# tud-amr/m3p2i-aip

Measured on AMD Instinct MI355X. Metric: mppi_state_steps_per_sec (K x T per command()), higher is better.
Workload: dtype f32; 1 GPU; point_env task=push goal=[-1.0, -1.0] K=2000 (2000/GPU) T=30 single-mode halton-spline, initial scene, open loop (fixed world, warm-started plan); parallelism=single GPU

## Files before the change

### include/m3p2i_hip.h

```cpp
#ifndef M3P2I_HIP_H
#define M3P2I_HIP_H

#ifdef __cplusplus
extern "C" {
#endif

#define M3_MAX_NU 9
#define M3_TOPK 20
#define M3_ABI_VERSION 4

typedef enum {
    M3_OK = 0,
    M3_ERR_BAD_ARG = -1,
    M3_ERR_HIP = -2,
    M3_ERR_SHAPE = -3,
    M3_ERR_STATE = -4,
    M3_ERR_UNSUPPORTED = -5
} m3_status;

typedef enum { M3_ENV_POINT = 0, M3_ENV_PANDA = 1 } m3_env;

typedef enum {
    M3_TASK_NAVIGATION = 0,
    M3_TASK_PUSH = 1,
// ... 86 lines not shown
    M3_BUF_PENDING_FORCE = 19,
    M3_BUF_INFO = 20,
    M3_BUF_SIM_WORLD = 21,
    M3_BUF_RECORD = 22,
    M3_BUF_RECORDS_ALL = 23,
    M3_BUF_NOISE_ALL = 24,
    M3_BUF_COV = 25,
    M3_BUF_RECORD_B = 26,
    M3_BUF_RECORDS_B_ALL = 27,
    M3_BUF_COUNT = 28
} m3_buffer_id;

typedef struct m3_handle m3_handle;

int m3_abi_version(void);
const char* m3_last_error(const m3_handle* h);
const char* m3_build_id(void);
void m3_default_config(m3_config* cfg, int env_type);
int m3_create(const m3_config* cfg, m3_handle** out);
void m3_destroy(m3_handle* h);
int m3_set_stream(m3_handle* h, void* hip_stream);
int m3_enable_timing(m3_handle* h, int on);
int m3_set_rollout_lanes(m3_handle* h, int lanes);
int m3_set_panda_lanes_per_sample(m3_handle* h, int lanes_per_sample);
int m3_set_panda_reach_cost_kernel(m3_handle* h, int on);
int m3_panda_lanes_per_sample_used(m3_handle* h);
int m3_panda_near_share(m3_handle* h);
int m3_set_update_launches(m3_handle* h, int launches);

int m3_set_wave_order(m3_handle* h, int on);
int m3_set_ladder_spins(m3_handle* h, int spins);
int m3_relabel_samples(m3_handle* h);

int m3_set_noise(m3_handle* h, const float* delta, int on_device);
int m3_set_noise_knots(m3_handle* h, const float* knots, int n_knots, int degree, float smoothing,
                       int on_device);
int m3_set_noise_global(m3_handle* h, const float* delta_all, int on_device);
int m3_set_noise_knots_global(m3_handle* h, const float* knots_all, int n_knots, int degree, float smoothing,
                              int on_device);
int m3_set_noise_halton(m3_handle* h, int n_knots, int degree, float smoothing);
#define M3_HALTON_PLAIN 0
#define M3_HALTON_FAURE 1
int m3_set_noise_halton_scrambled(m3_handle* h, int n_knots, int degree, float smoothing, int scramble);
int m3_sample_noise(m3_handle* h);
int m3_set_objective(m3_handle* h, int task, const float* goal, int goal_len, int gripper_cmd);
int m3_set_avoid_dyn_obs(m3_handle* h, int on);
// ... 137 lines not shown
```

### m3p2i_aip_amd/_lib.py

```python
from __future__ import annotations

import ctypes as C
import os

MAX_NU = 9
TOPK = 20
ABI_VERSION = 4

_HERE = os.path.dirname(os.path.abspath(__file__))
LIB_PATH = os.environ.get("M3P2I_HIP_LIB") or os.path.join(_HERE, "lib", "libm3p2i_hip.so")

ENV_POINT, ENV_PANDA = 0, 1
HALTON_PLAIN, HALTON_FAURE = 0, 1
IPC_HANDLE_BYTES = 64
TASKS = {"navigation": 0, "push": 1, "pull": 2, "push_pull": 3, "reach": 4, "pick": 5,
         "place": 6, "idle": 7}

(BUF_STATES, BUF_ACTIONS, BUF_COST_HORIZON, BUF_TRAJ_COST, BUF_TRAJ_COST_ALL, BUF_WEIGHTS,
 BUF_WEIGHTS_1, BUF_WEIGHTS_2, BUF_MEAN, BUF_MEAN_1, BUF_MEAN_2, BUF_BEST, BUF_BEST_1,
 BUF_BEST_2, BUF_ACTION_OUT, BUF_TOP_IDX, BUF_TOP_TRAJS, BUF_REDUCE, BUF_NOISE,
 BUF_PENDING_FORCE, BUF_INFO, BUF_SIM_WORLD, BUF_RECORD, BUF_RECORDS_ALL, BUF_NOISE_ALL, BUF_COV,
 BUF_RECORD_B, BUF_RECORDS_B_ALL, BUF_COUNT) = range(29)


# ... 57 lines not shown

PE_RUNNING, PE_SETTLING, PE_FROZEN = 0, 1, 2
PANDA_EPISODE_TRACE_FLOATS = 132
PE_TR_DOF, PE_TR_ROOT, PE_TR_ACTION, PE_TR_HAND, PE_TR_CUBE = 0, 18, 109, 118, 125


class Timing(C.Structure):
    _fields_ = [("rollout_ms", C.c_float), ("update_ms", C.c_float),
                ("finalize_ms", C.c_float), ("total_ms", C.c_float)]


_H = C.c_void_p
_FP = C.c_void_p
SYMBOLS = [
    ("m3_abi_version", C.c_int, []),
    ("m3_build_id", C.c_char_p, []),
    ("m3_last_error", C.c_char_p, [_H]),
    ("m3_default_config", None, [C.POINTER(Config), C.c_int]),
    ("m3_create", C.c_int, [C.POINTER(Config), C.POINTER(_H)]),
    ("m3_destroy", None, [_H]),
    ("m3_set_stream", C.c_int, [_H, C.c_void_p]),
    ("m3_enable_timing", C.c_int, [_H, C.c_int]),
    ("m3_set_rollout_lanes", C.c_int, [_H, C.c_int]),
    ("m3_set_panda_lanes_per_sample", C.c_int, [_H, C.c_int]),
    ("m3_panda_lanes_per_sample_used", C.c_int, [_H]),
    ("m3_panda_near_share", C.c_int, [_H]),
    ("m3_set_panda_reach_cost_kernel", C.c_int, [_H, C.c_int]),
    ("m3_set_update_launches", C.c_int, [_H, C.c_int]),
    ("m3_set_ladder_spins", C.c_int, [_H, C.c_int]),
    ("m3_set_wave_order", C.c_int, [_H, C.c_int]),
    ("m3_relabel_samples", C.c_int, [_H]),
    ("m3_set_noise", C.c_int, [_H, _FP, C.c_int]),
    ("m3_set_noise_knots", C.c_int, [_H, _FP, C.c_int, C.c_int, C.c_float, C.c_int]),
    ("m3_set_noise_global", C.c_int, [_H, _FP, C.c_int]),
    ("m3_set_noise_knots_global", C.c_int, [_H, _FP, C.c_int, C.c_int, C.c_float, C.c_int]),
    ("m3_set_noise_halton", C.c_int, [_H, C.c_int, C.c_int, C.c_float]),
    ("m3_set_noise_halton_scrambled", C.c_int, [_H, C.c_int, C.c_int, C.c_float, C.c_int]),
    ("m3_sample_noise", C.c_int, [_H]),
    ("m3_set_call_count", C.c_int, [_H, C.c_uint]),
    ("m3_set_objective", C.c_int, [_H, C.c_int, C.POINTER(C.c_float), C.c_int, C.c_int]),
    ("m3_set_avoid_dyn_obs", C.c_int, [_H, C.c_int]),
    ("m3_default_point_cost_weights", None, [C.POINTER(PointCostWeights)]),
    ("m3_set_point_cost_weights", C.c_int, [_H, C.POINTER(PointCostWeights)]),
    ("m3_get_point_cost_weights", C.c_int, [_H, C.POINTER(PointCostWeights)]),
    ("m3_set_weighted_cost_instance", C.c_int, [_H, C.c_int]),
    ("m3_set_multi_modal", C.c_int, [_H, C.c_int]),
# ... 104 lines not shown
```

### m3p2i_aip_amd/csrc/m3_api.hip

```cpp
#include <algorithm>
#include <cmath>
#include <cstddef>
#include <cstdio>
#include <cstdlib>
#include <cstring>
#include <tuple>
#include <vector>
#include <new>

#include "m3_internal.hpp"
#include "panda_episode_lane.hpp"

using namespace m3;

static thread_local std::string g_create_err;

#define HIPCHK(o, expr)                                                                  \
    do {                                                                                 \
        hipError_t e_ = (expr);                                                          \
        if (e_ != hipSuccess) {                                                          \
            (o)->err = std::string(#expr) + ": " + hipGetErrorString(e_);                \
            return M3_ERR_HIP;                                                           \
        }                                                                                \
    } while (0)
// ... 238 lines not shown
        if (hipMalloc((void**)&h->wave_min, (size_t)Kl * 3 * f) != hipSuccess) rc = M3_ERR_HIP;
        if (rc == M3_OK && hipMalloc((void**)&h->lflag, nl * sizeof(int)) != hipSuccess) rc = M3_ERR_HIP;
        if (rc == M3_OK && hipMemset(h->lflag, 0, nl * sizeof(int)) != hipSuccess) rc = M3_ERR_HIP;
    }
    if (rc == M3_OK && c->env_type == M3_ENV_PANDA) {
        void* p = nullptr;
        void* q = nullptr;
        void* d = nullptr;
        if (hipHostMalloc(&p, sizeof(int), hipHostMallocMapped) != hipSuccess || hipMalloc(&q, sizeof(unsigned long long)) != hipSuccess ||
            hipMemset(q, 0, sizeof(unsigned long long)) != hipSuccess || hipHostGetDevicePointer(&d, p, 0) != hipSuccess) {
            if (p) (void)hipHostFree(p);
            if (q) (void)hipFree(q);
            h->err = "m3_create: the panda rollout's report word (mapped host memory) could not be allocated";
            rc = M3_ERR_HIP;
        } else {
            h->panda_busy_hint = (int*)p;
            h->panda_busy_hint_dev = (int*)d;
            h->panda_busy_count = (unsigned long long*)q;
            *h->panda_busy_hint = 0;
        }
        if (rc == M3_OK && Kl == Kg && Kg >= 2 && Kl <= PANDA_REACH_REC_MAX_K &&
            hipMalloc((void**)&h->panda_reach_rec, (size_t)T * REACH_REC * (size_t)Kl * f) != hipSuccess) rc = M3_ERR_HIP;
    }
    if (rc == M3_OK && hipMalloc((void**)&h->wcount, (size_t)(T + 2) * sizeof(int)) != hipSuccess) rc = M3_ERR_HIP;
    if (rc == M3_OK && hipMemset(h->wcount, 0, (size_t)(T + 2) * sizeof(int)) != hipSuccess) rc = M3_ERR_HIP;
    if (rc == M3_OK) {
        m3_info init;
        std::memset(&init, 0, sizeof(init));
        init.beta = init.beta_1 = init.beta_2 = 1.0f;
        if (hipMemcpy(h->buf[M3_BUF_INFO], &init, sizeof(init), hipMemcpyHostToDevice) != hipSuccess) rc = M3_ERR_HIP;
    }
    if (rc != M3_OK) {
        g_create_err = h->err.empty() ? "m3_create: device allocation failed" : h->err;
        m3_destroy(h);
        return rc;
    }
    (void)hipDeviceSynchronize();
    *out = h;
    return M3_OK;
}

extern "C" void m3_destroy(m3_handle* h) {
    if (!h) return;
    if (h->regen) h->buf[M3_BUF_TRAJ_COST] = h->buf[M3_BUF_NOISE] = h->buf[M3_BUF_NOISE_ALL] = nullptr;
    for (int i = 0; i < M3_BUF_COUNT; ++i)
        if (h->buf[i]) (void)hipFree(h->buf[i]);
    if (h->noise_all) (void)hipFree(h->noise_all);
    if (h->noise_mats) (void)hipFree(h->noise_mats);
    if (h->local_top_idx) (void)hipFree(h->local_top_idx);
    if (h->world0_dev) (void)hipFree(h->world0_dev);
    if (h->topk_cand) (void)hipFree(h->topk_cand);
    if (h->part_min) (void)hipFree(h->part_min);
    if (h->lad) (void)hipFree(h->lad);
    if (h->wpart) (void)hipFree(h->wpart);
    if (h->apart) (void)hipFree(h->apart);
    if (h->wcount) (void)hipFree(h->wcount);
    if (h->wave_min) (void)hipFree(h->wave_min);
    if (h->lflag) (void)hipFree(h->lflag);
    if (h->sim_world) (void)hipFree(h->sim_world);
    if (h->sim_u) (void)hipFree(h->sim_u);
    if (h->noise_stage) (void)hipFree(h->noise_stage);
    if (h->order) (void)hipFree(h->order);
    if (h->order_scratch) (void)hipFree(h->order_scratch);
    if (h->noise_sorted) (void)hipFree(h->noise_sorted);
    for (int p = 0; p < MIX_MAX_RANKS; ++p)
        if (h->peer_ipc[p] && h->peer_base[p]) (void)hipIpcCloseMemHandle(h->peer_base[p]);
    if (h->xb) (void)hipFree(h->xb);
    if (h->panda_busy_hint) (void)hipHostFree(h->panda_busy_hint);
    if (h->panda_busy_count) (void)hipFree(h->panda_busy_count);
    if (h->panda_reach_rec) (void)hipFree(h->panda_reach_rec);
    for (auto& ev : h->ev)
        if (ev) (void)hipEventDestroy(ev);
    delete h;
}

#ifndef M3_BUILD_ID
#define M3_BUILD_ID "unknown"
#endif
extern "C" const char* m3_build_id(void) { return M3_BUILD_ID; }

extern "C" int m3_set_stream(m3_handle* h, void* s) {
    if (!h) return M3_ERR_BAD_ARG;
    h->stream = (hipStream_t)s;
    return M3_OK;
}

extern "C" int m3_set_rollout_lanes(m3_handle* h, int lanes) {
    if (!h) return M3_ERR_BAD_ARG;
    if (lanes != 0 && (lanes < 1 || lanes > 64 || (lanes & (lanes - 1)) != 0))
        return fail(h, M3_ERR_BAD_ARG, "m3_set_rollout_lanes: lanes must be 0 (auto) or a power of two in 1..64");
    h->lanes_override = lanes;
    return M3_OK;
}

extern "C" int m3_set_panda_lanes_per_sample(m3_handle* h, int lps) {
    if (!h) return M3_ERR_BAD_ARG;
    if (lps != 0 && lps != 1 && lps != 8 && lps != 16)
        return fail(h, M3_ERR_BAD_ARG, "m3_set_panda_lanes_per_sample: 0 (by size), 1, 8 or 16");
    h->panda_lps = lps;
    return M3_OK;
}

extern "C" int m3_set_panda_reach_cost_kernel(m3_handle* h, int on) {
    if (!h) return M3_ERR_BAD_ARG;
    h->panda_reach_deferred = on != 0;
    return M3_OK;
}

extern "C" int m3_panda_near_share(m3_handle* h) {
    return (h && h->panda_busy_hint) ? *(volatile const int*)h->panda_busy_hint - 1 : -1;
}

extern "C" int m3_panda_lanes_per_sample_used(m3_handle* h) {
    return h ? h->panda_lps_used : 0;
}
// ... 548 lines not shown
    a.cost_h = (float*)h->buf[M3_BUF_COST_HORIZON];
    a.J = (float*)h->buf[M3_BUF_TRAJ_COST];
    a.wave_min = h->wave_min;
    return M3_OK;
}

static void fill_panda_args(m3_handle* h, const RolloutArgs& a, PandaArgs& pa) {
    std::memcpy(pa.world0, h->pworld0, sizeof(pa.world0));
    pa.cubeA_actor = h->bind_box; pa.cubeB_actor = h->bind_dyn; pa.obs_actor = h->bind_obs;
    fill_panda_cost_params(h, pa.cp);
    pa.shadows = (pa.cp.task == 4 && a.k0 == 0 && a.Kl == a.Kg && a.Kg >= 2) ? (pa.cp.multi_modal ? 2 : 1) : 0;
    pa.lps = h->panda_lps;
    pa.reach_rec = (pa.shadows != 0 && a.Kl <= PANDA_REACH_REC_MAX_K && h->panda_reach_deferred) ? h->panda_reach_rec : nullptr;
    pa.busy_hint = h->panda_busy_hint_dev; pa.busy_count = h->panda_busy_count; pa.reach_busy = 0;
    if (h->panda_busy_hint) {
        const int share = *(volatile const int*)h->panda_busy_hint - 1;
        const int on = pa.reach_rec ? PANDA_BUSY_ON_REC : PANDA_BUSY_ON, off = pa.reach_rec ? PANDA_BUSY_OFF_REC : PANDA_BUSY_OFF;
        if (share >= on) h->panda_reach_busy = 1;
        else if (share >= 0 && share < off) h->panda_reach_busy = 0;
        pa.reach_busy = h->panda_reach_busy;
    }
}

static int plan_rollout(m3_handle* h, RolloutArgs& a, PandaArgs& pa, RolloutPlan& p) {
    const int rc = prepare_rollout(h, a);
    if (rc != M3_OK) return rc;
    if (h->cfg.env_type == M3_ENV_POINT) {
        p = plan_rollout_point(a, h->scene, weighted_cost(h));
    } else {
        fill_panda_args(h, a, pa);
        p = plan_rollout_panda(a, pa);
        h->panda_lps_used = p.lps;
    }
    a.lanes = p.lanes;
    h->wave_min_rows = p.rows;
    return M3_OK;
}

extern "C" int m3_rollout(m3_handle* h) {
    if (!h) return M3_ERR_BAD_ARG;
    if (const char* why = rollout_refusal(h)) return fail(h, M3_ERR_STATE, why);
    RolloutArgs a;
    PandaArgs pa;
    RolloutPlan p;
    const int rc = plan_rollout(h, a, pa, p);
    if (rc != M3_OK) return rc;
    if (h->timing) HIPCHK(h, hipEventRecord(h->ev[0], h->stream));
    if (h->cfg.env_type == M3_ENV_POINT) launch_rollout_point(a, h->scene, h->cost_weights, p, h->stream);
    else launch_rollout_panda(a, pa, h->pscene, p, h->stream);
    HIPCHK(h, hipGetLastError());
    if (h->timing) HIPCHK(h, hipEventRecord(h->ev[1], h->stream));
    return M3_OK;
}

static float* plan_dst(const m3_handle* h) { return h->action_out ? h->action_out : (float*)h->buf[M3_BUF_ACTION_OUT]; }
static size_t plan_floats(const m3_config& c) { return (size_t)(c.mode_simple ? c.u_per_command : c.T) * c.nu; }

static void fill_update_args(m3_handle* h, UpdateArgs& a) {
    const m3_config& c = h->cfg;
    std::memset(&a, 0, sizeof(a));
    a.Kg = c.K_global; a.Kl = c.K_local; a.k0 = c.k_offset; a.T = c.T; a.nu = c.nu;
    a.multi_modal = c.multi_modal; a.mode_simple = c.mode_simple; a.env_type = c.env_type;
    a.filter_u = c.filter_u; a.u_per_command = c.u_per_command;
    a.lambda_ = c.lambda_; a.step_size_mean = c.step_size_mean;
    a.cand = h->topk_cand;
    a.ladder_spins = h->ladder_spins;
    a.p2p_err = (h->p2p_ready && h->xb) ? (const int*)((const char*)h->xb + 2 * MIX_MAX_RANKS * sizeof(int)) : nullptr;
    a.part_min = h->part_min;
    a.n_cand = topk_workgroups(c.K_global);
    a.n_mins = mins_workgroups(c.K_global);
    a.lad = h->lad;
// ... 1441 lines not shown
```

### m3p2i_aip_amd/csrc/m3_internal.hpp

```cpp
#pragma once
#include <hip/hip_runtime.h>

#include <string>

#include "../../include/m3p2i_hip.h"
#include "planar_dyn.hpp"
#include "point_cost.hpp"
#include "panda_dyn.hpp"

namespace m3 {

struct RolloutArgs {
    int Kg, Kl, k0, T, nu;
    int multi_modal, mode_simple, sampling_random, sample_null_action;
    int gripper_cmd;
    float u_min[M3_MAX_NU], u_max[M3_MAX_NU], scale_tril[M3_MAX_NU], sigma_inv[M3_MAX_NU];
    float u_scale, gamma, lambda_;
    int noise_abs_cost, full_sigma;
    float noise_mu[M3_MAX_NU];
    const float* noise_mats;
    const float* scale_dev;
    unsigned long long seed;
    unsigned call;
    CostParams cp;
// ... 104 lines not shown

struct BatchRolloutEntry {
    RolloutArgs a;
    PointScene sc;
};
struct BatchRolloutEntryW {
    RolloutArgs a;
    PointScene sc;
    PointCostWeights wt;
};
struct SmallUpdateInstance {
    int nu, multi, jr, wt, n_cand;
};
SmallUpdateInstance update_small_instance(const UpdateArgs& a);
int update_small_batch_blocks_per_cu(const SmallUpdateInstance& in);
int update_small9_batch_blocks_per_cu(const SmallUpdateInstance& in);
void launch_update_small_batch(const UpdateArgs* tab, int n, const SmallUpdateInstance& in, int T, hipStream_t s);
struct RolloutPlan {
    int instance, ref;
    int lps, forces, general, shadows, rec;
    int lanes, blocks;
    int rows;
    int weighted;
};
RolloutPlan plan_rollout_point(const RolloutArgs& a, const PointScene& sc, bool weighted);
void launch_rollout_point_batch(const BatchRolloutEntry* tab, int n, const RolloutPlan& p, hipStream_t s);
void launch_rollout_point_batch_w(const BatchRolloutEntryW* tab, int n, const RolloutPlan& p, hipStream_t s);
void launch_rollout_point_nav_batch(const BatchRolloutEntry* tab, int blocks, int n, bool ref, hipStream_t s);
void launch_rollout_point_push_batch(const BatchRolloutEntry* tab, int blocks, int n, bool ref, hipStream_t s);
void launch_rollout_point_pull_batch(const BatchRolloutEntry* tab, int blocks, int n, bool ref, hipStream_t s);
void launch_rollout_point_pushpull_batch(const BatchRolloutEntry* tab, int blocks, int n, bool ref, hipStream_t s);

void launch_rollout_point(const RolloutArgs& a, const PointScene& sc, const PointCostWeights& wt ,
                          const RolloutPlan& p, hipStream_t s);
void launch_rollout_point_nav(const RolloutArgs& a, const PointScene& sc, int blocks, hipStream_t s);
void launch_rollout_point_push(const RolloutArgs& a, const PointScene& sc, int blocks, hipStream_t s);
void launch_rollout_point_pull(const RolloutArgs& a, const PointScene& sc, int blocks, hipStream_t s);
void launch_rollout_point_pushpull(const RolloutArgs& a, const PointScene& sc, int blocks, hipStream_t s);
void launch_transpose_noise(const float* src_ktn, float* dst_tkn, int K, int T, int nu,
                            hipStream_t s);
void launch_spline_noise(const float* knots, float* noise, int Kl, int nu, int n_knots, int T, int degree,
                         double smoothing, hipStream_t s);
void launch_sample_noise(const RolloutArgs& a, float* out, hipStream_t s);
void launch_halton_knots(float* knots, int k0, int n, int ncol, const int* primes_dev, const int* perm_dev,
                         const int* perm_off_dev, hipStream_t s);
struct OrderScene {
    const float* sim_root;
    int sim_box, sim_dyn;
    float bx, by, dx, dy;
    float ox, oy;
};
size_t wave_order_temp_bytes(int Kl);
hipError_t launch_wave_order(const float* noise, int Kl, int T, int nu, float s0, float s1, int half_local,
                             const OrderScene& os, void* scratch, size_t temp_bytes, int* order, float* noise_sorted,
                             const int* specials , hipStream_t s);
void launch_gather_rows(const float* src, const int* order, float* dst, int Kl, int rows, hipStream_t s);
void launch_weights(const UpdateArgs& a, hipStream_t s);
void launch_wsum(const UpdateArgs& a, hipStream_t s);
void launch_update_small(const UpdateArgs& a, hipStream_t s);
bool update_small_applies(const UpdateArgs& a);
void launch_finalize(const UpdateArgs& a, hipStream_t s);
void launch_mix(const UpdateArgs& a, hipStream_t s);
void launch_cov_update(const float* actions, const float* w, const float* mean, float* part, float* cov, int K, int T,
                       int nu, hipStream_t s);
void launch_local_topk(const UpdateArgs& a, hipStream_t s);
void launch_regen_fast(const UpdateArgs& a, hipStream_t s);
void launch_p3_search(const UpdateArgs& a, hipStream_t s);
void launch_p3_local_weights(const UpdateArgs& a, hipStream_t s);
void launch_p3_done(const UpdateArgs& a, hipStream_t s);
int init_ladder_table();
int regen_chunks(int Kg);
int rollout_lanes_for(int Kl);
constexpr int M3_CUS = 256;
constexpr int M3_SIMDS = 1024;
inline bool rollout_two_waves(int wavefronts) { return wavefronts > M3_SIMDS; }
inline bool rollout_three_waves(int wavefronts) { return wavefronts > 4 * M3_SIMDS; }
int mins_workgroups(int Kg);
int topk_workgroups(int Kg);
int ladder_workgroups(int Kg);
int wsum_chunks(int Kl);
int apply_workgroups(int Kg);
void launch_mins(const UpdateArgs& a, hipStream_t s);
void launch_ladder(const UpdateArgs& a, hipStream_t s);
void launch_ladder_search(const UpdateArgs& a, hipStream_t s);
void launch_fused_large(const UpdateArgs& a, hipStream_t s);

struct P2PArgs {
    const float* rec;
    int rec_len, rec_stride, n_ranks, rank, slot, seq;
    int plain_memory;
    unsigned long long timeout_ticks;
    int* err;
    float* peer_data[MIX_MAX_RANKS];
    int* peer_flags[MIX_MAX_RANKS];
};
constexpr size_t P2P_HDR_BYTES = 1024;
void launch_p2p_put(const P2PArgs& a, hipStream_t s);
void launch_p2p_wait(const P2PArgs& a, hipStream_t s);
void launch_p2p_exchange(const P2PArgs& a, hipStream_t s);
// ... 108 lines not shown
    int task = M3_TASK_PUSH;
    float goal[7] = {0, 0, 0, 0, 0, 0, 1};
    int gripper_cmd = 0;
    int avoid_dyn_obs = 0;
    m3::PointCostWeights cost_weights = m3::POINT_COST_WEIGHTS_DEFAULT;
    int weighted_instance = -1;
    float world0[18];
    const float* world0_bound = nullptr;
    const float* bind_dof = nullptr;
    const float* bind_root = nullptr;
    int bind_nact = 0, bind_box = 0, bind_dyn = 0, bind_obs = 0;
    bool have_noise = false;
    bool cov_active = false;
    float* noise_mats = nullptr;
    bool regen = false;
    bool regen_fast = false;
    bool p3 = false;
    const float* recb_src = nullptr;
    int recb_stride = 0;
    float* noise_all = nullptr;
    int* local_top_idx = nullptr;
    unsigned calls = 0;
    int lanes_override = 0;
    int* panda_busy_hint = nullptr;
    int* panda_busy_hint_dev = nullptr;
    unsigned long long* panda_busy_count = nullptr;
    float* panda_reach_rec = nullptr;
    bool panda_reach_deferred = true;
    int panda_reach_busy = 0;
    int panda_lps_used = 0;
    int panda_lps = 0;
    void* buf[M3_BUF_COUNT] = {};
    long long nbytes[M3_BUF_COUNT] = {};
    float* world0_dev = nullptr;
    float* action_out = nullptr;
    m3::VI* topk_cand = nullptr;
    float* part_min = nullptr;
    float* lad = nullptr;
    float* wpart = nullptr;
    float* apart = nullptr;
    int* wcount = nullptr;
    float* wave_min = nullptr;
    int wave_min_rows = 0;
    bool use_wave_min = false;
    int* lflag = nullptr;
    int lad_epoch = 0;
// ... 22 lines not shown
```

### m3p2i_aip_amd/csrc/rollout_point.hip

```cpp
#include "rollout_point_kernel.hpp"
#include "episode_lane.hpp"

namespace m3 {

int rollout_lanes_for(int Kl) {
    (void)Kl;
    return 64;
}

__global__ __launch_bounds__(64) void k_rollout_point_w(const RolloutArgs a, const PointScene sc, const PointCostWeights wt) {
    rollout_point_body<true, -1, true, true>(a, sc, &wt);
}
__global__ __launch_bounds__(64) void k_rollout_point_w_ref(const RolloutArgs a, const PointCostWeights wt) {
    constexpr PointScene sc = POINT_SCENE_REFERENCE;
    rollout_point_body<true, -1, true, true>(a, sc, &wt);
}
__global__ __launch_bounds__(64) __attribute__((amdgpu_waves_per_eu(2, 2))) void k_rollout_point_w_occ2(
    const RolloutArgs a, const PointScene sc, const PointCostWeights wt) {
    rollout_point_body<true, -1, false, true>(a, sc, &wt);
}
__global__ __launch_bounds__(64) __attribute__((amdgpu_waves_per_eu(3, 3))) void k_rollout_point_w_occ3(
    const RolloutArgs a, const PointScene sc, const PointCostWeights wt) {
    rollout_point_body<true, -1, false, true>(a, sc, &wt);
}
// ... 11 lines not shown
}
__global__ __launch_bounds__(64) void kb_rollout_point_w_ref(const BatchRolloutEntryW* __restrict__ tab) {
    constexpr PointScene sc = POINT_SCENE_REFERENCE;
    rollout_point_body<true, -1, true, true>(tab[blockIdx.y].a, sc, &tab[blockIdx.y].wt);
}
__global__ __launch_bounds__(64) __attribute__((amdgpu_waves_per_eu(2, 2))) void kb_rollout_point_w_occ2(
    const BatchRolloutEntryW* __restrict__ tab) {
    rollout_point_body<true, -1, false, true>(tab[blockIdx.y].a, tab[blockIdx.y].sc, &tab[blockIdx.y].wt);
}
__global__ __launch_bounds__(64) __attribute__((amdgpu_waves_per_eu(3, 3))) void kb_rollout_point_w_occ3(
    const BatchRolloutEntryW* __restrict__ tab) {
    rollout_point_body<true, -1, false, true>(tab[blockIdx.y].a, tab[blockIdx.y].sc, &tab[blockIdx.y].wt);
}
static void launch_rollout_point_weighted_batch(const BatchRolloutEntryW* tab, int blocks, int n, bool ref, hipStream_t s) {
    const dim3 grid(blocks, n);
    switch (rollout_point_build(blocks * n, ref)) {
        case BUILD_OCC3: hipLaunchKernelGGL(kb_rollout_point_w_occ3, grid, dim3(64), 0, s, tab); break;
        case BUILD_OCC2: hipLaunchKernelGGL(kb_rollout_point_w_occ2, grid, dim3(64), 0, s, tab); break;
        case BUILD_LONE_REF: hipLaunchKernelGGL(kb_rollout_point_w_ref, grid, dim3(64), 0, s, tab); break;
        default: hipLaunchKernelGGL(kb_rollout_point_w, grid, dim3(64), 0, s, tab); break;
    }
}

RolloutPlan plan_rollout_point(const RolloutArgs& a, const PointScene& sc, bool weighted) {
#if defined(M3_ABL_GENERAL_ONLY) || defined(M3_ABL_COUNT) || defined(M3_ABL_PHASES)
    const bool general = true;
#else
    const bool general = a.sampling_random || a.mode_simple || a.cp.task < 0 || a.cp.task > 3 ||
                         (a.cp.task == 3 && !a.multi_modal) || a.scale_dev != nullptr  ||
                         a.cp.avoid_dyn_obs != 0  ||
                         weighted ;
#endif
    RolloutPlan p{};
    p.weighted = weighted ? 1 : 0;
    p.instance = general ? -1 : a.cp.task;
    p.ref = point_scene_is_reference(sc) ? 1 : 0;
    p.lanes = a.lanes;
    p.blocks = (a.Kl + a.lanes - 1) / a.lanes;
    p.rows = (a.wave_min && (p.instance == -1 || p.instance == 3)) ? p.blocks : 0;
    return p;
}

void launch_rollout_point(const RolloutArgs& a, const PointScene& sc, const PointCostWeights& wt, const RolloutPlan& p,
                          hipStream_t s) {
    if (p.weighted) { launch_rollout_point_weighted(a, sc, wt, p.blocks, s); return; }
    switch (p.instance) {
        case -1: launch_rollout_point_instance<true, -1>(a, sc, p.blocks, s); break;
        case 0: launch_rollout_point_nav(a, sc, p.blocks, s); break;
        case 1: launch_rollout_point_push(a, sc, p.blocks, s); break;
        case 2: launch_rollout_point_pull(a, sc, p.blocks, s); break;
        default: launch_rollout_point_pushpull(a, sc, p.blocks, s); break;
    }
}

void launch_rollout_point_batch(const BatchRolloutEntry* tab, int n, const RolloutPlan& p, hipStream_t s) {
    const bool ref = p.ref != 0;
    switch (p.instance) {
        case -1: launch_rollout_point_batch_instance<true, -1>(tab, p.blocks, n, ref, s); break;
        case 0: launch_rollout_point_nav_batch(tab, p.blocks, n, ref, s); break;
        case 1: launch_rollout_point_push_batch(tab, p.blocks, n, ref, s); break;
        case 2: launch_rollout_point_pull_batch(tab, p.blocks, n, ref, s); break;
        default: launch_rollout_point_pushpull_batch(tab, p.blocks, n, ref, s); break;
    }
}

void launch_rollout_point_batch_w(const BatchRolloutEntryW* tab, int n, const RolloutPlan& p, hipStream_t s) {
    launch_rollout_point_weighted_batch(tab, p.blocks, n, p.ref != 0, s);
}
// ... 316 lines not shown
```

### m3p2i_aip_amd/csrc/rollout_point_kernel.hpp

```cpp
#pragma once
#include "m3_internal.hpp"
#include "noise_stream.hpp"
#include "wave_min.hpp"

namespace m3 {

__device__ __forceinline__ void load_world(const float* p, PointWorld& w) {
    w.rx = p[0]; w.ry = p[1]; w.rvx = p[2]; w.rvy = p[3];
    w.B.x = p[4]; w.B.y = p[5]; w.B.c = p[6]; w.B.s = p[7]; w.B.vx = p[8]; w.B.vy = p[9]; w.B.w = p[10];
    w.D.x = p[11]; w.D.y = p[12]; w.D.c = p[13]; w.D.s = p[14]; w.D.vx = p[15]; w.D.vy = p[16]; w.D.w = p[17];
    w.fcDx = w.fcDy = w.fcBx = w.fcBy = w.fcRx = w.fcRy = 0.0f;
}

__device__ __forceinline__ void load_world_from_sim(const float* dof, const float* root, int box,
                                                    int dyn, PointWorld& w) {
    w.rx = dof[0]; w.ry = dof[2]; w.rvx = dof[1]; w.rvy = dof[3];
    const float* r = root + (size_t)box * 13;
    float qz = r[5], qw = r[6];
    w.B.x = r[0]; w.B.y = r[1]; w.B.c = 1.0f - 2.0f * (qz * qz); w.B.s = 2.0f * (qz * qw);
    w.B.vx = r[7]; w.B.vy = r[8]; w.B.w = r[12];
    r = root + (size_t)dyn * 13;
    qz = r[5]; qw = r[6];
    w.D.x = r[0]; w.D.y = r[1]; w.D.c = 1.0f - 2.0f * (qz * qz); w.D.s = 2.0f * (qz * qw);
    w.D.vx = r[7]; w.D.vy = r[8]; w.D.w = r[12];
// ... 142 lines not shown
    rollout_point_body<GENERAL, TASK, false>(a, sc);
}
template <bool GENERAL, int TASK>
__global__ __launch_bounds__(64) __attribute__((amdgpu_waves_per_eu(3, 3))) void k_rollout_point_occ3(const RolloutArgs a,
                                                                                                      const PointScene sc) {
    rollout_point_body<GENERAL, TASK, false>(a, sc);
}
enum RolloutBuild { BUILD_LONE, BUILD_LONE_REF, BUILD_OCC2, BUILD_OCC3 };
inline RolloutBuild rollout_point_build(int waves, bool ref) {
    if (rollout_three_waves(waves)) return BUILD_OCC3;
    if (rollout_two_waves(waves)) return BUILD_OCC2;
    return ref ? BUILD_LONE_REF : BUILD_LONE;
}
template <bool GENERAL, int TASK>
inline void launch_rollout_point_instance(const RolloutArgs& a, const PointScene& sc, int blocks, hipStream_t s) {
    switch (rollout_point_build(blocks, point_scene_is_reference(sc))) {
        case BUILD_OCC3: hipLaunchKernelGGL((k_rollout_point_occ3<GENERAL, TASK>), dim3(blocks), dim3(64), 0, s, a, sc); break;
        case BUILD_OCC2: hipLaunchKernelGGL((k_rollout_point_occ2<GENERAL, TASK>), dim3(blocks), dim3(64), 0, s, a, sc); break;
        case BUILD_LONE_REF: hipLaunchKernelGGL((k_rollout_point_ref<GENERAL, TASK>), dim3(blocks), dim3(64), 0, s, a); break;
        default: hipLaunchKernelGGL((k_rollout_point<GENERAL, TASK>), dim3(blocks), dim3(64), 0, s, a, sc); break;
    }
}

template <bool GENERAL, int TASK>
__global__ __launch_bounds__(64) void kb_rollout_point(const BatchRolloutEntry* __restrict__ tab) {
    rollout_point_body<GENERAL, TASK>(tab[blockIdx.y].a, tab[blockIdx.y].sc);
}
template <bool GENERAL, int TASK>
__global__ __launch_bounds__(64) void kb_rollout_point_ref(const BatchRolloutEntry* __restrict__ tab) {
    constexpr PointScene sc = POINT_SCENE_REFERENCE;
    rollout_point_body<GENERAL, TASK>(tab[blockIdx.y].a, sc);
}
template <bool GENERAL, int TASK>
__global__ __launch_bounds__(64) __attribute__((amdgpu_waves_per_eu(2, 2))) void kb_rollout_point_occ2(
    const BatchRolloutEntry* __restrict__ tab) {
    rollout_point_body<GENERAL, TASK, false>(tab[blockIdx.y].a, tab[blockIdx.y].sc);
}
template <bool GENERAL, int TASK>
__global__ __launch_bounds__(64) __attribute__((amdgpu_waves_per_eu(3, 3))) void kb_rollout_point_occ3(
    const BatchRolloutEntry* __restrict__ tab) {
    rollout_point_body<GENERAL, TASK, false>(tab[blockIdx.y].a, tab[blockIdx.y].sc);
}
template <bool GENERAL, int TASK>
inline void launch_rollout_point_batch_instance(const BatchRolloutEntry* tab, int blocks, int n, bool ref, hipStream_t s) {
    const dim3 grid(blocks, n);
    switch (rollout_point_build(blocks * n, ref)) {
// ... 9 lines not shown
```

### m3p2i_aip_amd/csrc/rollout_point_task0.hip

```cpp
#include "rollout_point_kernel.hpp"

namespace m3 {

void launch_rollout_point_nav(const RolloutArgs& a, const PointScene& sc, int blocks, hipStream_t s) {
    launch_rollout_point_instance<false, 0>(a, sc, blocks, s);
}
void launch_rollout_point_nav_batch(const BatchRolloutEntry* tab, int blocks, int n, bool ref, hipStream_t s) {
    launch_rollout_point_batch_instance<false, 0>(tab, blocks, n, ref, s);
}

}
```

### m3p2i_aip_amd/csrc/rollout_point_task1.hip

```cpp
#include "rollout_point_kernel.hpp"

namespace m3 {

void launch_rollout_point_push(const RolloutArgs& a, const PointScene& sc, int blocks, hipStream_t s) {
    launch_rollout_point_instance<false, 1>(a, sc, blocks, s);
}
void launch_rollout_point_push_batch(const BatchRolloutEntry* tab, int blocks, int n, bool ref, hipStream_t s) {
    launch_rollout_point_batch_instance<false, 1>(tab, blocks, n, ref, s);
}

}
```

### m3p2i_aip_amd/engine.py

```python
from __future__ import annotations

import os

import ctypes as C

import numpy as np
import torch

from . import _lib as L


class _DevArray:

    def __init__(self, ptr, shape, typestr, owner):
        self.__cuda_array_interface__ = {"shape": tuple(shape), "typestr": typestr,
                                         "data": (int(ptr), False), "version": 2}
        self._owner = owner


def make_config(K, T, nu=2, env_type="point_env", multi_modal=False, mode_simple=False,
                sampling_random=False, sample_null_action=True, filter_u=True,
                u_per_command=None, u_min=None, u_max=None, noise_sigma_diag=None, u_scale=1.0,
                gamma=0.95, lambda_=1.0, kp_suction=400.0, pre_height_diff=0.05, dt=None,
                substeps=2, solver_iters=6, seed=0, device=0, K_local=None, k_offset=0,
# ... 41 lines not shown
    c.seed = int(seed)
    return c


class HipEngine:
    def __init__(self, cfg: L.Config):
        if not torch.cuda.is_available():
            raise L.M3Error("HipEngine needs a HIP device (torch.cuda.is_available() is False); "
                            "there is no CPU fallback")
        self.lib = L.load()
        self.cfg = cfg
        self._h = C.c_void_p()
        torch.cuda.set_device(cfg.device)
        torch.zeros(1, device=f"cuda:{cfg.device}")
        L.check(self.lib.m3_create(C.byref(cfg), C.byref(self._h)))
        self.device = torch.device(f"cuda:{cfg.device}")
        self._views = {}
        self._action_out = None
        self.use_torch_stream()
        if os.environ.get("M3P2I_WAVE_ORDER", "1") == "0":
            self.set_wave_order(False)
        if os.environ.get("M3P2I_ROLLOUT_LANES"):
            self.set_rollout_lanes(int(os.environ["M3P2I_ROLLOUT_LANES"]))

    def close(self):
        if getattr(self, "_h", None) is not None and self._h:
            self._views.clear()
            self.lib.m3_destroy(self._h)
            self._h = C.c_void_p()

    def __del__(self):
        try:
            self.close()
        except Exception:
            pass

    def _ck(self, rc):
        L.check(rc, self._h)

    def use_torch_stream(self, stream=None):
        s = stream if stream is not None else torch.cuda.current_stream(self.device)
        self._ck(self.lib.m3_set_stream(self._h, C.c_void_p(s.cuda_stream)))

    def set_rollout_lanes(self, lanes=0):
        self._ck(self.lib.m3_set_rollout_lanes(self._h, int(lanes)))

    def set_panda_lanes_per_sample(self, lps=0):
        self._ck(self.lib.m3_set_panda_lanes_per_sample(self._h, int(lps)))

    def panda_lanes_per_sample_used(self):
        return int(self.lib.m3_panda_lanes_per_sample_used(self._h))

    def set_panda_reach_cost_kernel(self, on=True):
        self._ck(self.lib.m3_set_panda_reach_cost_kernel(self._h, int(bool(on))))

    def panda_near_share(self):
        return int(self.lib.m3_panda_near_share(self._h))

    def set_update_launches(self, launches=0):
        self._ck(self.lib.m3_set_update_launches(self._h, int(launches)))

    def set_ladder_spins(self, spins=-1):
        self._ck(self.lib.m3_set_ladder_spins(self._h, int(spins)))

    def set_wave_order(self, on=True):
        self._ck(self.lib.m3_set_wave_order(self._h, int(bool(on))))

    def relabel_samples(self):
# ... 502 lines not shown
```

Baseline: 512.7 million state-steps/s.

## Split point rollout into producer/consumer wavefronts handing off through LDS

Adds a two-wavefront form of the point-env rollout kernel for navigation and push. One wavefront computes controls and writes actions while the other steps the dynamics serially, and that same control wavefront then evaluates costs and writes states from LDS behind the dynamics wavefront, using atomic progress counters. The aim is to take control construction, cost evaluation and global stores off the serial dynamics chain so they overlap with it. The form is picked automatically when blocks are few (K=2000 here). A mapped-host error word records spin timeouts, which adds a host read per call and a risk of invalid results if a wait runs out.

```diff
diff --git a/include/m3p2i_hip.h b/include/m3p2i_hip.h
--- a/include/m3p2i_hip.h
+++ b/include/m3p2i_hip.h
@@ -132,6 +132,8 @@
 int m3_set_stream(m3_handle* h, void* hip_stream);
 int m3_enable_timing(m3_handle* h, int on);
 int m3_set_rollout_lanes(m3_handle* h, int lanes);
+int m3_set_point_rollout_form(m3_handle* h, int form);
+int m3_point_rollout_form_used(m3_handle* h);
 int m3_set_panda_lanes_per_sample(m3_handle* h, int lanes_per_sample);
 int m3_set_panda_reach_cost_kernel(m3_handle* h, int on);
 int m3_panda_lanes_per_sample_used(m3_handle* h);
diff --git a/m3p2i_aip_amd/_lib.py b/m3p2i_aip_amd/_lib.py
--- a/m3p2i_aip_amd/_lib.py
+++ b/m3p2i_aip_amd/_lib.py
@@ -103,6 +103,8 @@
     ("m3_set_stream", C.c_int, [_H, C.c_void_p]),
     ("m3_enable_timing", C.c_int, [_H, C.c_int]),
     ("m3_set_rollout_lanes", C.c_int, [_H, C.c_int]),
+    ("m3_set_point_rollout_form", C.c_int, [_H, C.c_int]),
+    ("m3_point_rollout_form_used", C.c_int, [_H]),
     ("m3_set_panda_lanes_per_sample", C.c_int, [_H, C.c_int]),
     ("m3_panda_lanes_per_sample_used", C.c_int, [_H]),
     ("m3_panda_near_share", C.c_int, [_H]),
diff --git a/m3p2i_aip_amd/csrc/m3_api.hip b/m3p2i_aip_amd/csrc/m3_api.hip
--- a/m3p2i_aip_amd/csrc/m3_api.hip
+++ b/m3p2i_aip_amd/csrc/m3_api.hip
@@ -284,6 +284,19 @@
         if (rc == M3_OK && Kl == Kg && Kg >= 2 && Kl <= PANDA_REACH_REC_MAX_K &&
             hipMalloc((void**)&h->panda_reach_rec, (size_t)T * REACH_REC * (size_t)Kl * f) != hipSuccess) rc = M3_ERR_HIP;
     }
+    if (rc == M3_OK && c->env_type == M3_ENV_POINT && !c->sim_only) {
+        void* p = nullptr;
+        void* d = nullptr;
+        if (hipHostMalloc(&p, sizeof(int), hipHostMallocMapped) != hipSuccess || hipHostGetDevicePointer(&d, p, 0) != hipSuccess) {
+            if (p) (void)hipHostFree(p);
+            h->err = "m3_create: the point rollout's error word (mapped host memory) could not be allocated";
+            rc = M3_ERR_HIP;
+        } else {
+            h->rollout_err = (int*)p;
+            h->rollout_err_dev = (int*)d;
+            *h->rollout_err = 0;
+        }
+    }
     if (rc == M3_OK && hipMalloc((void**)&h->wcount, (size_t)(T + 2) * sizeof(int)) != hipSuccess) rc = M3_ERR_HIP;
     if (rc == M3_OK && hipMemset(h->wcount, 0, (size_t)(T + 2) * sizeof(int)) != hipSuccess) rc = M3_ERR_HIP;
     if (rc == M3_OK) {
@@ -329,6 +342,7 @@
         if (h->peer_ipc[p] && h->peer_base[p]) (void)hipIpcCloseMemHandle(h->peer_base[p]);
     if (h->xb) (void)hipFree(h->xb);
     if (h->panda_busy_hint) (void)hipHostFree(h->panda_busy_hint);
+    if (h->rollout_err) (void)hipHostFree(h->rollout_err);
     if (h->panda_busy_count) (void)hipFree(h->panda_busy_count);
     if (h->panda_reach_rec) (void)hipFree(h->panda_reach_rec);
     for (auto& ev : h->ev)
@@ -353,6 +367,17 @@
         return fail(h, M3_ERR_BAD_ARG, "m3_set_rollout_lanes: lanes must be 0 (auto) or a power of two in 1..64");
     h->lanes_override = lanes;
     return M3_OK;
+}
+
+extern "C" int m3_set_point_rollout_form(m3_handle* h, int form) {
+    if (!h) return M3_ERR_BAD_ARG;
+    if (form < -1 || form > 1) return fail(h, M3_ERR_BAD_ARG, "m3_set_point_rollout_form: 0 (one wavefront), 1 (two) or -1 (automatic)");
+    h->point_form = form;
+    return M3_OK;
+}
+
+extern "C" int m3_point_rollout_form_used(m3_handle* h) {
+    return h ? h->point_form_used : -1;
 }
 
 extern "C" int m3_set_panda_lanes_per_sample(m3_handle* h, int lps) {
@@ -947,11 +972,11 @@
     }
 }
 
-static int plan_rollout(m3_handle* h, RolloutArgs& a, PandaArgs& pa, RolloutPlan& p) {
+static int plan_rollout(m3_handle* h, RolloutArgs& a, PandaArgs& pa, RolloutPlan& p, bool own_launch = false) {
     const int rc = prepare_rollout(h, a);
     if (rc != M3_OK) return rc;
     if (h->cfg.env_type == M3_ENV_POINT) {
-        p = plan_rollout_point(a, h->scene, weighted_cost(h));
+        p = plan_rollout_point(a, h->scene, weighted_cost(h), (own_launch && h->rollout_err_dev) ? h->point_form : 0);
     } else {
         fill_panda_args(h, a, pa);
         p = plan_rollout_panda(a, pa);
@@ -968,10 +993,14 @@
     RolloutArgs a;
     PandaArgs pa;
     RolloutPlan p;
-    const int rc = plan_rollout(h, a, pa, p);
+    if (h->rollout_err && *(volatile const int*)h->rollout_err != 0)
+        return fail(h, M3_ERR_HIP, "m3_rollout: a hand-over wait between the two wavefronts of an earlier rollout launch ran out "
+                                   "(its results are invalid); m3_set_point_rollout_form(h, 0) avoids the form");
+    const int rc = plan_rollout(h, a, pa, p, true);
     if (rc != M3_OK) return rc;
+    if (h->cfg.env_type == M3_ENV_POINT) h->point_form_used = p.form;
     if (h->timing) HIPCHK(h, hipEventRecord(h->ev[0], h->stream));
-    if (h->cfg.env_type == M3_ENV_POINT) launch_rollout_point(a, h->scene, h->cost_weights, p, h->stream);
+    if (h->cfg.env_type == M3_ENV_POINT) launch_rollout_point(a, h->scene, h->cost_weights, p, h->stream, h->rollout_err_dev);
     else launch_rollout_panda(a, pa, h->pscene, p, h->stream);
     HIPCHK(h, hipGetLastError());
     if (h->timing) HIPCHK(h, hipEventRecord(h->ev[1], h->stream));
diff --git a/m3p2i_aip_amd/csrc/m3_internal.hpp b/m3p2i_aip_amd/csrc/m3_internal.hpp
--- a/m3p2i_aip_amd/csrc/m3_internal.hpp
+++ b/m3p2i_aip_amd/csrc/m3_internal.hpp
@@ -150,8 +150,9 @@
     int lanes, blocks;
     int rows;
     int weighted;
-};
-RolloutPlan plan_rollout_point(const RolloutArgs& a, const PointScene& sc, bool weighted);
+    int form;
+};
+RolloutPlan plan_rollout_point(const RolloutArgs& a, const PointScene& sc, bool weighted, int form_request = 0);
 void launch_rollout_point_batch(const BatchRolloutEntry* tab, int n, const RolloutPlan& p, hipStream_t s);
 void launch_rollout_point_batch_w(const BatchRolloutEntryW* tab, int n, const RolloutPlan& p, hipStream_t s);
 void launch_rollout_point_nav_batch(const BatchRolloutEntry* tab, int blocks, int n, bool ref, hipStream_t s);
@@ -160,7 +161,9 @@
 void launch_rollout_point_pushpull_batch(const BatchRolloutEntry* tab, int blocks, int n, bool ref, hipStream_t s);
 
 void launch_rollout_point(const RolloutArgs& a, const PointScene& sc, const PointCostWeights& wt ,
-                          const RolloutPlan& p, hipStream_t s);
+                          const RolloutPlan& p, hipStream_t s, int* err = nullptr );
+void launch_rollout_point_nav2(const RolloutArgs& a, const PointScene& sc, int blocks, int* err, hipStream_t s);
+void launch_rollout_point_push2(const RolloutArgs& a, const PointScene& sc, int blocks, int* err, hipStream_t s);
 void launch_rollout_point_nav(const RolloutArgs& a, const PointScene& sc, int blocks, hipStream_t s);
 void launch_rollout_point_push(const RolloutArgs& a, const PointScene& sc, int blocks, hipStream_t s);
 void launch_rollout_point_pull(const RolloutArgs& a, const PointScene& sc, int blocks, hipStream_t s);
@@ -203,6 +206,12 @@
 constexpr int M3_SIMDS = 1024;
 inline bool rollout_two_waves(int wavefronts) { return wavefronts > M3_SIMDS; }
 inline bool rollout_three_waves(int wavefronts) { return wavefronts > 4 * M3_SIMDS; }
+constexpr int ROLLOUT_COMPANION_MAX_BLOCKS = M3_SIMDS / 2;
+inline bool rollout_companion_pays(int blocks) { return blocks <= ROLLOUT_COMPANION_MAX_BLOCKS; }
+constexpr int R2_COMPS = 8;
+constexpr size_t R2_LDS_MAX = 64 * 1024;
+inline size_t rollout_point2_lds_bytes(int T) { return 16 + (size_t)T * R2_COMPS * 64 * sizeof(float); }
+inline bool rollout_point2_fits(int T) { return T >= 1 && rollout_point2_lds_bytes(T) <= R2_LDS_MAX; }
 int mins_workgroups(int Kg);
 int topk_workgroups(int Kg);
 int ladder_workgroups(int Kg);
@@ -357,6 +366,10 @@
     int* local_top_idx = nullptr;
     unsigned calls = 0;
     int lanes_override = 0;
+    int point_form = -1;
+    int point_form_used = -1;
+    int* rollout_err = nullptr;
+    int* rollout_err_dev = nullptr;
     int* panda_busy_hint = nullptr;
     int* panda_busy_hint_dev = nullptr;
     unsigned long long* panda_busy_count = nullptr;
diff --git a/m3p2i_aip_amd/csrc/rollout_point.hip b/m3p2i_aip_amd/csrc/rollout_point.hip
--- a/m3p2i_aip_amd/csrc/rollout_point.hip
+++ b/m3p2i_aip_amd/csrc/rollout_point.hip
@@ -57,7 +57,7 @@
     }
 }
 
-RolloutPlan plan_rollout_point(const RolloutArgs& a, const PointScene& sc, bool weighted) {
+RolloutPlan plan_rollout_point(const RolloutArgs& a, const PointScene& sc, bool weighted, int form_request) {
 #if defined(M3_ABL_GENERAL_ONLY) || defined(M3_ABL_COUNT) || defined(M3_ABL_PHASES)
     const bool general = true;
 #else
@@ -73,12 +73,21 @@
     p.lanes = a.lanes;
     p.blocks = (a.Kl + a.lanes - 1) / a.lanes;
     p.rows = (a.wave_min && (p.instance == -1 || p.instance == 3)) ? p.blocks : 0;
+    const RolloutBuild build = rollout_point_build(p.blocks, p.ref != 0);
+    const bool exists = (p.instance == 0 || p.instance == 1) && !weighted && (build == BUILD_LONE || build == BUILD_LONE_REF) &&
+                        rollout_point2_fits(a.T);
+    p.form = (exists && (form_request == 1 || (form_request < 0 && rollout_companion_pays(p.blocks)))) ? 1 : 0;
     return p;
 }
 
 void launch_rollout_point(const RolloutArgs& a, const PointScene& sc, const PointCostWeights& wt, const RolloutPlan& p,
-                          hipStream_t s) {
+                          hipStream_t s, int* err) {
     if (p.weighted) { launch_rollout_point_weighted(a, sc, wt, p.blocks, s); return; }
+    if (p.form == 1) {
+        if (p.instance == 0) launch_rollout_point_nav2(a, sc, p.blocks, err, s);
+        else launch_rollout_point_push2(a, sc, p.blocks, err, s);
+        return;
+    }
     switch (p.instance) {
         case -1: launch_rollout_point_instance<true, -1>(a, sc, p.blocks, s); break;
         case 0: launch_rollout_point_nav(a, sc, p.blocks, s); break;
diff --git a/m3p2i_aip_amd/csrc/rollout_point_kernel.hpp b/m3p2i_aip_amd/csrc/rollout_point_kernel.hpp
--- a/m3p2i_aip_amd/csrc/rollout_point_kernel.hpp
+++ b/m3p2i_aip_amd/csrc/rollout_point_kernel.hpp
@@ -188,6 +188,138 @@
     }
 }
 
+constexpr unsigned R2_SPINS_DYN = 1u << 16;
+constexpr unsigned R2_SPINS_COMP = 1u << 16;
+__device__ __forceinline__ unsigned r2_peek(const unsigned* word) {
+    return __builtin_amdgcn_readfirstlane(__hip_atomic_load(word, __ATOMIC_RELAXED, __HIP_MEMORY_SCOPE_WORKGROUP));
+}
+template <int TASK>
+__device__ __forceinline__ void rollout_point_body2(const RolloutArgs& a_, const PointScene& sc, int* err) {
+    static_assert(TASK == 0 || TASK == 1, "the cost of pull / push_pull stages the suction force of the next step");
+    extern __shared__ __attribute__((aligned(16))) float r2_lds[];
+    RolloutArgs a = a_;
+    a.sampling_random = 0; a.mode_simple = 0;
+    a.noise_abs_cost = 0; a.full_sigma = 0; a.scale_dev = nullptr;
+    a.cp.avoid_dyn_obs = 0;
+    a.cp.task = TASK;
+    unsigned* const words = reinterpret_cast<unsigned*>(r2_lds);
+    float* const tab = r2_lds + 4;
+    const int wave = __builtin_amdgcn_readfirstlane((int)threadIdx.x >> 6);
+    const int lane = (int)threadIdx.x & 63;
+    if (threadIdx.x == 0) { words[0] = 0u; words[1] = 0u; }
+    __syncthreads();
+    const int slot = blockIdx.x * a.lanes + lane;
+    if (lane >= a.lanes || slot >= a.Kl) return;
+    const int i = a.order ? a.order[slot] : slot;
+    const int Kl = a.Kl, T = a.T;
+    const int k = a.k0 + i;
+#define M3_R2(t, c) tab[((t) * R2_COMPS + (c)) * 64 + lane]
+    if (wave == 0) {
+        PointWorld w;
+        if (a.sim_dof) load_world_from_sim(a.sim_dof, a.sim_root, a.sim_box, a.sim_dyn, w);
+        else load_world(a.world0, w);
+        w.fRx = a.pend[0 * Kl + i]; w.fRy = a.pend[1 * Kl + i];
+        w.fBx = a.pend[2 * Kl + i]; w.fBy = a.pend[3 * Kl + i];
+        unsigned ready = 0u;
+        bool ok = true;
+        auto controls = [&](int t, float& u0, float& u1) {
+            if (ready < (unsigned)(t + 1)) {
+                for (unsigned spins = 0u; (ready = r2_peek(&words[0])) < (unsigned)(t + 1);)
+                    if (++spins > R2_SPINS_DYN) { *err = 1; ok = false; break; }
+                __builtin_amdgcn_fence(__ATOMIC_ACQUIRE, "workgroup");
+            }
+            u0 = M3_R2(t, 6); u1 = M3_R2(t, 7);
+        };
+        float n0, n1;
+        controls(0, n0, n1);
+        for (int t = 0; t < T && ok; ++t) {
+            const float u0 = n0, u1 = n1;
+            if (t + 1 < T) controls(t + 1, n0, n1);
+            point_step<false, true>(sc, w, u0, u1, TASK == 0);
+            M3_R2(t, 0) = w.rx; M3_R2(t, 1) = w.rvx; M3_R2(t, 2) = w.ry; M3_R2(t, 3) = w.rvy;
+            if constexpr (TASK == 0) { M3_R2(t, 4) = w.fcDx; M3_R2(t, 5) = w.fcDy; }
+            else { M3_R2(t, 4) = w.B.x; M3_R2(t, 5) = w.B.y; }
+            __hip_atomic_store(&words[1], (unsigned)(t + 1), __ATOMIC_RELEASE, __HIP_MEMORY_SCOPE_WORKGROUP);
+        }
+        a.pend[0 * Kl + i] = w.fRx; a.pend[1 * Kl + i] = w.fRy;
+        a.pend[2 * Kl + i] = w.fBx; a.pend[3 * Kl + i] = w.fBy;
+    } else {
+        const bool is_last = (k == a.Kg - 1);
+        const bool first_half = k < a.cp.half_K;
+        const float* mptr = a.mean;
+        if (a.multi_modal) mptr = first_half ? a.mean1 : a.mean2;
+        struct StepIn { float d0, d1, m0, m1, b0, b1; };
+        const bool use_best = a.multi_modal && (k == 0 || k == a.cp.half_K);
+        const float* bptr = (k == 0) ? a.best1 : a.best2;
+        auto fetch = [&](int t) {
+            StepIn in;
+            in.b0 = in.b1 = 0.0f;
+            const float2 dd = *reinterpret_cast<const float2*>(a.delta + ((size_t)t * Kl + slot) * 2);
+            in.d0 = dd.x; in.d1 = dd.y;
+            const int ts = (t + 1 < T) ? t + 1 : T - 1;
+            in.m0 = mptr[ts * 2 + 0]; in.m1 = mptr[ts * 2 + 1];
+            if (use_best) { in.b0 = bptr[ts * 2 + 0]; in.b1 = bptr[ts * 2 + 1]; }
+            return in;
+        };
+        StepIn nxt = fetch(0);
+        for (int t = 0; t < T; ++t) {
+            const StepIn in = nxt;
+            if (t + 1 < T) nxt = fetch(t + 1);
+            float d0 = in.d0, d1 = in.d1;
+            if (is_last) { d0 = 0.0f; d1 = 0.0f; }
+            float a0 = fmaxf(fminf(in.m0 + d0 * a.scale_tril[0], a.u_max[0]), a.u_min[0]);
+            float a1 = fmaxf(fminf(in.m1 + d1 * a.scale_tril[1], a.u_max[1]), a.u_min[1]);
+            if (use_best) { a0 = in.b0; a1 = in.b1; }
+            float u0 = a.u_scale * a0, u1 = a.u_scale * a1;
+            if (a.sample_null_action && is_last) { u0 = 0.0f; u1 = 0.0f; }
+            M3_R2(t, 6) = u0; M3_R2(t, 7) = u1;
+            __hip_atomic_store(&words[0], (unsigned)(t + 1), __ATOMIC_RELEASE, __HIP_MEMORY_SCOPE_WORKGROUP);
+            *reinterpret_cast<float2*>(a.actions + ((size_t)t * Kl + i) * 2) = make_float2(u0, u1);
+        }
+        float J = 0.0f, S = 0.0f, g = 1.0f;
+        unsigned recorded = 0u;
+        PointWorld w = {};
+        for (int t = 0; t < T; ++t) {
+            if (recorded < (unsigned)(t + 1)) {
+                bool ok = true;
+                for (unsigned spins = 0u; (recorded = r2_peek(&words[1])) < (unsigned)(t + 1);) {
+                    if (++spins > R2_SPINS_COMP) { *err = 2; ok = false; break; }
+                    __builtin_amdgcn_s_sleep(4);
+                }
+                if (!ok) break;
+                __builtin_amdgcn_fence(__ATOMIC_ACQUIRE, "workgroup");
+            }
+            w.rx = M3_R2(t, 0); w.rvx = M3_R2(t, 1); w.ry = M3_R2(t, 2); w.rvy = M3_R2(t, 3);
+            if constexpr (TASK == 0) { w.fcDx = M3_R2(t, 4); w.fcDy = M3_R2(t, 5); }
+            else { w.B.x = M3_R2(t, 4); w.B.y = M3_R2(t, 5); }
+            const float c = point_cost(a.cp, w, k);
+            *reinterpret_cast<float4*>(a.states + ((size_t)t * Kl + i) * 4) =
+                make_float4(w.rx, w.rvx, w.ry, w.rvy);
+            a.cost_h[(size_t)t * Kl + i] = c;
+            J = J + g * c;
+            S = S + c;
+            g = g * a.gamma;
+        }
+        a.J[i] = J;
+    }
+#undef M3_R2
+}
+template <int TASK>
+__global__ __launch_bounds__(128) void k_rollout_point2(const RolloutArgs a, const PointScene sc, int* err) {
+    rollout_point_body2<TASK>(a, sc, err);
+}
+template <int TASK>
+__global__ __launch_bounds__(128) void k_rollout_point2_ref(const RolloutArgs a, int* err) {
+    constexpr PointScene sc = POINT_SCENE_REFERENCE;
+    rollout_point_body2<TASK>(a, sc, err);
+}
+template <int TASK>
+inline void launch_rollout_point2_instance(const RolloutArgs& a, const PointScene& sc, int blocks, int* err, hipStream_t s) {
+    const size_t lds = rollout_point2_lds_bytes(a.T);
+    if (point_scene_is_reference(sc)) hipLaunchKernelGGL((k_rollout_point2_ref<TASK>), dim3(blocks), dim3(128), lds, s, a, err);
+    else hipLaunchKernelGGL((k_rollout_point2<TASK>), dim3(blocks), dim3(128), lds, s, a, sc, err);
+}
+
 template <bool GENERAL, int TASK>
 __global__ __launch_bounds__(64) void kb_rollout_point(const BatchRolloutEntry* __restrict__ tab) {
     rollout_point_body<GENERAL, TASK>(tab[blockIdx.y].a, tab[blockIdx.y].sc);
diff --git a/m3p2i_aip_amd/csrc/rollout_point_task0.hip b/m3p2i_aip_amd/csrc/rollout_point_task0.hip
--- a/m3p2i_aip_amd/csrc/rollout_point_task0.hip
+++ b/m3p2i_aip_amd/csrc/rollout_point_task0.hip
@@ -5,6 +5,9 @@
 void launch_rollout_point_nav(const RolloutArgs& a, const PointScene& sc, int blocks, hipStream_t s) {
     launch_rollout_point_instance<false, 0>(a, sc, blocks, s);
 }
+void launch_rollout_point_nav2(const RolloutArgs& a, const PointScene& sc, int blocks, int* err, hipStream_t s) {
+    launch_rollout_point2_instance<0>(a, sc, blocks, err, s);
+}
 void launch_rollout_point_nav_batch(const BatchRolloutEntry* tab, int blocks, int n, bool ref, hipStream_t s) {
     launch_rollout_point_batch_instance<false, 0>(tab, blocks, n, ref, s);
 }
diff --git a/m3p2i_aip_amd/csrc/rollout_point_task1.hip b/m3p2i_aip_amd/csrc/rollout_point_task1.hip
--- a/m3p2i_aip_amd/csrc/rollout_point_task1.hip
+++ b/m3p2i_aip_amd/csrc/rollout_point_task1.hip
@@ -5,6 +5,9 @@
 void launch_rollout_point_push(const RolloutArgs& a, const PointScene& sc, int blocks, hipStream_t s) {
     launch_rollout_point_instance<false, 1>(a, sc, blocks, s);
 }
+void launch_rollout_point_push2(const RolloutArgs& a, const PointScene& sc, int blocks, int* err, hipStream_t s) {
+    launch_rollout_point2_instance<1>(a, sc, blocks, err, s);
+}
 void launch_rollout_point_push_batch(const BatchRolloutEntry* tab, int blocks, int n, bool ref, hipStream_t s) {
     launch_rollout_point_batch_instance<false, 1>(tab, blocks, n, ref, s);
 }
diff --git a/m3p2i_aip_amd/engine.py b/m3p2i_aip_amd/engine.py
--- a/m3p2i_aip_amd/engine.py
+++ b/m3p2i_aip_amd/engine.py
@@ -87,6 +87,8 @@
             self.set_wave_order(False)
         if os.environ.get("M3P2I_ROLLOUT_LANES"):
             self.set_rollout_lanes(int(os.environ["M3P2I_ROLLOUT_LANES"]))
+        if os.environ.get("M3P2I_POINT_ROLLOUT_FORM"):
+            self.set_point_rollout_form(int(os.environ["M3P2I_POINT_ROLLOUT_FORM"]))
 
     def close(self):
         if getattr(self, "_h", None) is not None and self._h:
@@ -109,6 +111,12 @@
 
     def set_rollout_lanes(self, lanes=0):
         self._ck(self.lib.m3_set_rollout_lanes(self._h, int(lanes)))
+
+    def set_point_rollout_form(self, form=-1):
+        self._ck(self.lib.m3_set_point_rollout_form(self._h, int(form)))
+
+    def point_rollout_form_used(self):
+        return int(self.lib.m3_point_rollout_form_used(self._h))
 
     def set_panda_lanes_per_sample(self, lps=0):
         self._ck(self.lib.m3_set_panda_lanes_per_sample(self._h, int(lps)))
```

New measurement: 552.5 million state-steps/s (median of 6 runs). +7.8%, better.
